# Veason-silverbullet/DIGAT

Measured on NVIDIA B200. Metric: impressions_scored_per_sec, higher is better.
Workload: dtype f32

## Files before the change

### digat_b200/csrc/gemm_tcgen05_persistent.cuh

```cuda
#pragma once
#include "gemm_tcgen05.cuh"
#include "gemm_tcgen05_pair.cuh"

namespace digat {

__device__ __forceinline__ void tma_load_2d_multicast(void* dst, const CUtensorMap* map, uint64_t* bar, int c0, int c1,
                                                      uint16_t cta_mask) {
    asm volatile(
        "cp.async.bulk.tensor.2d.shared::cluster.global.mbarrier::complete_tx::bytes.multicast::cluster [%0], [%1, {%3, %4}], [%2], %5;"
        :: "r"(smem_u32(dst)), "l"(reinterpret_cast<uint64_t>(map)), "r"(smem_u32(bar)), "r"(c0), "r"(c1), "h"(cta_mask) : "memory");
}
__device__ __forceinline__ void umma_commit_multicast(uint64_t* bar, uint16_t cta_mask) {
    asm volatile("tcgen05.commit.cta_group::1.mbarrier::arrive::one.shared::cluster.multicast::cluster.b64 [%0], %1;"
                 :: "r"(smem_u32(bar)), "h"(cta_mask) : "memory");
}

__device__ __forceinline__ void umma_bf16_2cta(uint32_t tmem_d, uint64_t da, uint64_t db, uint32_t idesc, uint32_t accumulate) {
    asm volatile(
        "{\n\t.reg .pred p;\n\t"
        "setp.ne.b32 p, %4, 0;\n\t"
        "tcgen05.mma.cta_group::2.kind::f16 [%0], %1, %2, %3, p;\n\t}"
        :: "r"(tmem_d), "l"(da), "l"(db), "r"(idesc), "r"(accumulate) : "memory");
}

constexpr int kTcEpiWarps = 8;
constexpr int kTcPersistThreads = (2 + 4 + kTcEpiWarps) * 32;

template <int BN, int kCl = 1>
struct TcPersistCfg {
    static constexpr int A_BYTES = 128 * kTcBK * 4;
    static constexpr int W_ROWS = kCl == 3 ? BN / 2 : BN;
    static constexpr int W_BYTES = W_ROWS * kTcBK * 4;
    static constexpr int STAGE_BYTES = 2 * A_BYTES + 2 * W_BYTES;
    static constexpr int MAX_N = 1280;
    static constexpr int GB_GROUPS = 16;
    static constexpr int EXTRA = 512  + MAX_N * 4 + kTcEpiWarps * 32 * 20 * 4  + GB_GROUPS * BN * 4;
    static constexpr int STAGES = (226 * 1024 - EXTRA) / STAGE_BYTES > 6 ? 6 : (226 * 1024 - EXTRA) / STAGE_BYTES;
    static constexpr int TMEM_COLS = 2 * BN <= 256 ? 256 : 512;
    static constexpr size_t SMEM = (size_t)STAGES * STAGE_BYTES + EXTRA;
    static_assert(STAGES >= 3, "not enough shared memory for the pipeline");
    static_assert(A_BYTES % 512 == 0 && W_BYTES % 512 == 0, "operand tiles must start on a swizzle-atom boundary");
};

template <int BN, bool kBf16, int kCl>
__global__ void __launch_bounds__(kTcPersistThreads, 1)
gemm_tf32x3_persistent_kernel(const __grid_constant__ CUtensorMap map_a, const __grid_constant__ CUtensorMap map_whi,
                              const __grid_constant__ CUtensorMap map_wlo, const __grid_constant__ CUtensorMap map_w3,
                              const float* __restrict__ bias,
                              float* __restrict__ C, int ldc, int M, int N, int K, GroupBias gb) {
    using Cfg = TcPersistCfg<BN, kCl>;
    extern __shared__ __align__(1024) uint8_t smem_raw[];
    uint8_t* smem = smem_raw;
    uint64_t* bars = reinterpret_cast<uint64_t*>(smem + (size_t)Cfg::STAGES * Cfg::STAGE_BYTES);
    uint64_t* full = bars;
    uint64_t* ready = bars + Cfg::STAGES;
    uint64_t* empty = bars + 2 * Cfg::STAGES;
    uint64_t* accum_full = bars + 3 * Cfg::STAGES;
    uint64_t* tmem_empty = accum_full + 1;
    uint64_t* peer_full = tmem_empty + 1;
    uint32_t* tmem_slot = reinterpret_cast<uint32_t*>(peer_full + Cfg::STAGES);
    float* bias_s = reinterpret_cast<float*>(smem + (size_t)Cfg::STAGES * Cfg::STAGE_BYTES + 512);
    float* stage_base = bias_s + Cfg::MAX_N;
    float* gb_s = stage_base + kTcEpiWarps * 32 * 20;

    const int warp = threadIdx.x >> 5, lane = threadIdx.x & 31;
    const int nkb_all = (K + kTcBK - 1) / kTcBK;
    const int nkb = (nkb_all + gb.kbatches - 1) / gb.kbatches;
    const int n_tiles_n = (N + BN - 1) / BN, n_tiles_m = (M + 127) / 128;
    const int cl_rank = kCl >= 2 ? (int)cluster_ctarank() : 0;
    const int worker = kCl >= 2 ? (int)(blockIdx.x >> 1) : (int)blockIdx.x;
    const int n_workers = kCl >= 2 ? (int)(gridDim.x >> 1) : (int)gridDim.x;
    const int n_units_m = kCl >= 2 ? (n_tiles_m + 1) / 2 : n_tiles_m;
    const int n_tiles_mn = n_tiles_n * n_units_m;
    const int n_tiles = n_tiles_mn * gb.kbatches;
    auto tile_mb = [&](int t_mn) { const int u = t_mn / n_tiles_n; return kCl >= 2 ? 2 * u + cl_rank : u; };
    auto tile_nb = [&](int t_mn) { return t_mn % n_tiles_n; };

    auto a_hi = [&](int s) { return smem + (size_t)s * Cfg::STAGE_BYTES; };
    auto a_lo = [&](int s) { return smem + (size_t)s * Cfg::STAGE_BYTES + Cfg::A_BYTES; };
    auto w_hi = [&](int s) { return smem + (size_t)s * Cfg::STAGE_BYTES + 2 * Cfg::A_BYTES; };
    auto w_lo = [&](int s) { return smem + (size_t)s * Cfg::STAGE_BYTES + 2 * Cfg::A_BYTES + Cfg::W_BYTES; };
    auto a_b2 = [&](int s) { return a_lo(s) + Cfg::A_BYTES / 2; };
    auto w_b3 = [&](int s) { return w_lo(s) + Cfg::W_BYTES / 2; };

    for (int i = threadIdx.x; i < N; i += kTcPersistThreads) bias_s[i] = bias != nullptr ? bias[i] : 0.f;
    if (warp == 0 && lane == 0) {
        asm volatile("prefetch.tensormap [%0];" :: "l"(reinterpret_cast<uint64_t>(&map_a)) : "memory");
        asm volatile("prefetch.tensormap [%0];" :: "l"(reinterpret_cast<uint64_t>(&map_whi)) : "memory");
        asm volatile("prefetch.tensormap [%0];" :: "l"(reinterpret_cast<uint64_t>(&map_wlo)) : "memory");
        for (int s = 0; s < Cfg::STAGES; ++s) {
            mbar_init(&full[s], 1);
            mbar_init(&ready[s], kTcTransformThreads / 32 + ((kCl == 3 && cl_rank == 0) ? 1 : 0));
            mbar_init(&empty[s], kCl == 2 ? 2 : 1);
            mbar_init(&peer_full[s], 1);
        }
        mbar_init(accum_full, 1);
        mbar_init(tmem_empty, kCl == 3 ? 2 * kTcEpiWarps : kTcEpiWarps);
        asm volatile("fence.mbarrier_init.release.cluster;" ::: "memory");
    }
    if (warp == 1) {
        if (kCl == 3) {
            asm volatile("tcgen05.alloc.cta_group::2.sync.aligned.shared::cta.b32 [%0], %1;"
                         :: "r"(smem_u32(tmem_slot)), "r"((uint32_t)Cfg::TMEM_COLS) : "memory");
            asm volatile("tcgen05.relinquish_alloc_permit.cta_group::2.sync.aligned;" ::: "memory");
        } else {
            asm volatile("tcgen05.alloc.cta_group::1.sync.aligned.shared::cta.b32 [%0], %1;"
                         :: "r"(smem_u32(tmem_slot)), "r"((uint32_t)Cfg::TMEM_COLS) : "memory");
            asm volatile("tcgen05.relinquish_alloc_permit.cta_group::1.sync.aligned;" ::: "memory");
        }
    }
    asm volatile("tcgen05.fence::before_thread_sync;" ::: "memory");
    if (kCl >= 2) cluster_sync_all();
    else __syncthreads();
    asm volatile("tcgen05.fence::after_thread_sync;" ::: "memory");
    const uint32_t tmem_base = *tmem_slot;

    if (warp == 0) {
        if (lane == 0) {
            int it = 0;
            for (int tile = worker; tile < n_tiles; tile += n_workers) {
                const int slice = tile / n_tiles_mn, t_mn = tile - slice * n_tiles_mn;
                const int mb = tile_mb(t_mn), m0 = mb * 128, n0 = tile_nb(t_mn) * BN;
                const int kb0 = slice * nkb;
                if (n0 == 0 && gb.kbatches == 1) {
                    const int ahead = mb + kTcPrefetchBlocks;
                    if (ahead < n_tiles_m)
                        for (int kb = 0; kb < nkb; ++kb)
                            asm volatile("cp.async.bulk.prefetch.tensor.2d.L2.global [%0, {%1, %2}];"
                                         :: "l"(reinterpret_cast<uint64_t>(&map_a)), "r"(kb * kTcBK), "r"(ahead * 128) : "memory");
                }
                for (int kb = 0; kb < nkb; ++kb, ++it) {
                    const int s = it % Cfg::STAGES;
                    if (kCl >= 2) mbar_wait_cluster(&empty[s], ((it / Cfg::STAGES) & 1) ^ 1);
                    else mbar_wait(&empty[s], ((it / Cfg::STAGES) & 1) ^ 1);
                    mbar_arrive_expect_tx(&full[s], Cfg::A_BYTES + 2 * Cfg::W_BYTES);
                    tma_load_2d(a_hi(s), &map_a, &full[s], (kb0 + kb) * kTcBK, m0);
                    if (kCl == 2) {
                        constexpr int HR = BN / 2;
                        const int nr = n0 + cl_rank * HR;
                        tma_load_2d_multicast(w_hi(s) + cl_rank * HR * kTcBK * 4, &map_whi, &full[s], (kb0 + kb) * kTcBK, nr, 3);
                        tma_load_2d_multicast(w_lo(s) + cl_rank * HR * kTcBK * (kBf16 ? 2 : 4), &map_wlo, &full[s], (kb0 + kb) * kTcBK, nr, 3);
                        if (kBf16) tma_load_2d_multicast(w_b3(s) + cl_rank * HR * kTcBK * 2, &map_w3, &full[s], (kb0 + kb) * kTcBK, nr, 3);
                    } else {
                        const int nr = kCl == 3 ? n0 + cl_rank * (BN / 2) : n0;
                        tma_load_2d(w_hi(s), &map_whi, &full[s], (kb0 + kb) * kTcBK, nr);
                        tma_load_2d(w_lo(s), &map_wlo, &full[s], (kb0 + kb) * kTcBK, nr);
                        if (kBf16) tma_load_2d(w_b3(s), &map_w3, &full[s], (kb0 + kb) * kTcBK, nr);
                    }
                }
            }
        }
    } else if (warp == 1) {
        if (kCl == 3) {
            if (lane == 0 && cl_rank == 0) {
                constexpr uint32_t idesc2 = umma_idesc_tf32(256, BN);
                constexpr uint32_t idesc2h = umma_idesc_bf16(256, BN);
                const uint32_t d_main = tmem_base, d_corr = tmem_base + (uint32_t)BN;
                int it = 0, j = 0;
                for (int tile = worker; tile < n_tiles; tile += n_workers, ++j) {
                    if (j > 0) {
                        mbar_wait_cluster(tmem_empty, (uint32_t)(j - 1) & 1u);
                        asm volatile("tcgen05.fence::after_thread_sync;" ::: "memory");
                    }
                    auto issue_raw = [&](int kb, int g) {
                        const int s = g % Cfg::STAGES;
                        mbar_wait(&full[s], (g / Cfg::STAGES) & 1);
                        mbar_wait_cluster(&peer_full[s], (g / Cfg::STAGES) & 1);
                        asm volatile("tcgen05.fence::after_thread_sync;" ::: "memory");
                        const uint64_t d_ahi = umma_desc_sw64(smem_u32(a_hi(s)));
                        const uint64_t d_whi = umma_desc_sw64(smem_u32(w_hi(s))), d_wlo = umma_desc_sw64(smem_u32(w_lo(s)));
#pragma unroll
                        for (int k = 0; k < kTcBK / 8; ++k) {
                            const uint64_t koff = (uint64_t)((k * 8 * 4) >> 4);
                            const uint32_t first = (kb > 0 || k > 0) ? 1u : 0u;
                            umma_tf32_2cta(d_main, d_ahi + koff, d_whi + koff, idesc2, first);
                            if (!kBf16) umma_tf32_2cta(d_corr, d_ahi + koff, d_wlo + koff, idesc2, first);
                        }
                    };
                    auto issue_lo = [&](int g) {
                        const int s = g % Cfg::STAGES;
                        mbar_wait_cluster(&ready[s], (g / Cfg::STAGES) & 1);
                        asm volatile("tcgen05.fence::after_thread_sync;" ::: "memory");
                        if (kBf16) {
                            const uint32_t first = (g - it) > 0 ? 1u : 0u;
                            umma_bf16_2cta(d_corr, umma_desc_sw32(smem_u32(a_lo(s))), umma_desc_sw32(smem_u32(w_b3(s))), idesc2h, first);
                            umma_bf16_2cta(d_corr, umma_desc_sw32(smem_u32(a_b2(s))), umma_desc_sw32(smem_u32(w_lo(s))), idesc2h, 1u);
                        } else {
                            const uint64_t d_alo = umma_desc_sw64(smem_u32(a_lo(s))), d_whi = umma_desc_sw64(smem_u32(w_hi(s)));
#pragma unroll
                            for (int k = 0; k < kTcBK / 8; ++k) {
                                const uint64_t koff = (uint64_t)((k * 8 * 4) >> 4);
                                umma_tf32_2cta(d_corr, d_alo + koff, d_whi + koff, idesc2, 1u);
                            }
                        }
                        umma_commit_2cta(&empty[s]);
                    };
                    issue_raw(0, it);
                    for (int kb = 0; kb < nkb; ++kb) {
                        if (kb + 1 < nkb) issue_raw(kb + 1, it + kb + 1);
                        issue_lo(it + kb);
                    }
                    it += nkb;
                    umma_commit_2cta(accum_full);
                }
            } else if (cl_rank == 1 && lane < 2) {
                int it = 0;
                for (int tile = worker; tile < n_tiles; tile += n_workers)
                    for (int kb = 0; kb < nkb; ++kb, ++it) {
                        const int s = it % Cfg::STAGES;
                        if (lane == 0) {
                            mbar_wait(&full[s], (it / Cfg::STAGES) & 1);
                            mbar_arrive_cluster(&peer_full[s], 0);
                        } else {
                            mbar_wait(&ready[s], (it / Cfg::STAGES) & 1);
                            mbar_arrive_cluster(&ready[s], 0);
                        }
                    }
            }
        } else if (lane == 0) {
            constexpr uint32_t idesc = umma_idesc_tf32(128, BN);
            const uint32_t d_main = tmem_base, d_corr = tmem_base + (uint32_t)BN;
            int it = 0, j = 0;
            for (int tile = worker; tile < n_tiles; tile += n_workers, ++j) {
#ifdef DIGAT_TC_TIMING
                const long long t0 = clock64();
#endif
                if (j > 0) {
                    mbar_wait(tmem_empty, (uint32_t)(j - 1) & 1u);
                    asm volatile("tcgen05.fence::after_thread_sync;" ::: "memory");
                }
#ifdef DIGAT_TC_TIMING
                const long long t1 = clock64();
#endif
                auto issue_raw = [&](int kb, int g) {
                    const int s = g % Cfg::STAGES;
                    mbar_wait(&full[s], (g / Cfg::STAGES) & 1);
                    asm volatile("tcgen05.fence::after_thread_sync;" ::: "memory");
                    const uint64_t d_ahi = umma_desc_sw64(smem_u32(a_hi(s)));
                    const uint64_t d_whi = umma_desc_sw64(smem_u32(w_hi(s))), d_wlo = umma_desc_sw64(smem_u32(w_lo(s)));
#pragma unroll
                    for (int k = 0; k < kTcBK / 8; ++k) {
                        const uint64_t koff = (uint64_t)((k * 8 * 4) >> 4);
                        const uint32_t first = (kb > 0 || k > 0) ? 1u : 0u;
                        umma_tf32(d_main, d_ahi + koff, d_whi + koff, idesc, first);
                        if (!kBf16) umma_tf32(d_corr, d_ahi + koff, d_wlo + koff, idesc, first);
                    }
                };
                auto issue_lo = [&](int g) {
                    const int s = g % Cfg::STAGES;
                    mbar_wait(&ready[s], (g / Cfg::STAGES) & 1);
                    asm volatile("tcgen05.fence::after_thread_sync;" ::: "memory");
                    if (kBf16) {
                        constexpr uint32_t idesc16 = umma_idesc_bf16(128, BN);
                        const uint32_t first = (g - it) > 0 ? 1u : 0u;
                        umma_bf16(d_corr, umma_desc_sw32(smem_u32(a_lo(s))), umma_desc_sw32(smem_u32(w_b3(s))), idesc16, first);
                        umma_bf16(d_corr, umma_desc_sw32(smem_u32(a_b2(s))), umma_desc_sw32(smem_u32(w_lo(s))), idesc16, 1u);
                    } else {
                        const uint64_t d_alo = umma_desc_sw64(smem_u32(a_lo(s))), d_whi = umma_desc_sw64(smem_u32(w_hi(s)));
#pragma unroll
                        for (int k = 0; k < kTcBK / 8; ++k) {
                            const uint64_t koff = (uint64_t)((k * 8 * 4) >> 4);
                            umma_tf32(d_corr, d_alo + koff, d_whi + koff, idesc, 1u);
                        }
                    }
                    if (kCl == 2) umma_commit_multicast(&empty[s], 3);
                    else umma_commit(&empty[s]);
                };
                issue_raw(0, it);
                for (int kb = 0; kb < nkb; ++kb) {
                    if (kb + 1 < nkb) issue_raw(kb + 1, it + kb + 1);
                    issue_lo(it + kb);
                }
                it += nkb;
                umma_commit(accum_full);
#ifdef DIGAT_TC_TIMING
                if (blockIdx.x == 7 && j >= 3 && j <= 5)
                    printf("mma  tile j=%d: waited tmem_empty %lld, issue loop %lld (abs %lld)\n", j, t1 - t0, clock64() - t1, t0);
#endif
            }
        }
    } else if (warp < 6) {
        const int t = threadIdx.x - 64;
        int it = 0;
        for (int tile = worker; tile < n_tiles; tile += n_workers) {
            for (int kb = 0; kb < nkb; ++kb, ++it) {
                const int s = it % Cfg::STAGES;
                mbar_wait(&full[s], (it / Cfg::STAGES) & 1);
                const float4* hi = reinterpret_cast<const float4*>(a_hi(s));
                float4* lo = reinterpret_cast<float4*>(a_lo(s));
#pragma unroll
                for (int i = 0; i < Cfg::A_BYTES / 16 / kTcTransformThreads; ++i) {
                    const int idx = t + i * kTcTransformThreads;
                    const float4 v = hi[idx];
                    if (kBf16) {
                        const int r = idx >> 2, c = (idx & 3) ^ ((r >> 1) & 3);
                        const uint32_t off = (uint32_t)(r * 32 + (((c >> 1) ^ ((r >> 2) & 1)) << 4) + ((c & 1) << 3));
                        __nv_bfloat162 p0 = __floats2bfloat162_rn(v.x, v.y), p1 = __floats2bfloat162_rn(v.z, v.w);
                        __nv_bfloat162 q0 = __floats2bfloat162_rn(v.x - tf32_trunc(v.x), v.y - tf32_trunc(v.y));
                        __nv_bfloat162 q1 = __floats2bfloat162_rn(v.z - tf32_trunc(v.z), v.w - tf32_trunc(v.w));
                        uint2 full_v, lo_v;
                        full_v.x = *reinterpret_cast<uint32_t*>(&p0); full_v.y = *reinterpret_cast<uint32_t*>(&p1);
                        lo_v.x = *reinterpret_cast<uint32_t*>(&q0); lo_v.y = *reinterpret_cast<uint32_t*>(&q1);
                        *reinterpret_cast<uint2*>(a_lo(s) + off) = full_v;
                        *reinterpret_cast<uint2*>(a_b2(s) + off) = lo_v;
                    } else {
                        float4 vl;
                        vl.x = to_tf32_rna(v.x - tf32_trunc(v.x)); vl.y = to_tf32_rna(v.y - tf32_trunc(v.y));
                        vl.z = to_tf32_rna(v.z - tf32_trunc(v.z)); vl.w = to_tf32_rna(v.w - tf32_trunc(v.w));
                        lo[idx] = vl;
                    }
                }
                asm volatile("fence.proxy.async.shared::cta;" ::: "memory");
                __syncwarp();
                if (lane == 0) mbar_arrive(&ready[s]);
            }
        }
    } else {
        const int q = warp & 3;
        const int ew = warp - 6;
        const int c_begin = (kTcEpiWarps == 8 && ew >= 4) ? (BN > 128 ? 128 : BN) : 0;
        const int c_end = (kTcEpiWarps == 8 && ew < 4) ? (BN > 128 ? 128 : BN) : BN;
        const bool has_gb = gb.ptr != nullptr;
        float* stage = stage_base + ew * (32 * 20);
        const uint32_t tbase = tmem_base + ((uint32_t)(q * 32) << 16);
        int j = 0;
        for (int tile = worker; tile < n_tiles; tile += n_workers, ++j) {
            const int slice = tile / n_tiles_mn, t_mn = tile - slice * n_tiles_mn;
            const int mb = tile_mb(t_mn), m0 = mb * 128, n0 = tile_nb(t_mn) * BN;
            float* __restrict__ Cs = C + (size_t)slice * (size_t)gb.c_batch_stride;
            const int m = m0 + q * 32 + lane;
            const int32_t* orow = gb.out_rows;
            const int mo = orow != nullptr ? orow[min(m, M - 1)] : m;
            const int g0 = has_gb ? (orow != nullptr ? orow[m0] : m0) / gb.rows : 0;
            const int g1 = has_gb ? (orow != nullptr ? orow[min(m0 + 127, M - 1)] : min(m0 + 127, M - 1)) / gb.rows : 0;
            const bool gb_tile = has_gb && n0 < gb.col0 + gb.cols && n0 + BN > gb.col0;
            const bool gb_smem = gb_tile && (g1 - g0 + 1) <= Cfg::GB_GROUPS;
            if (gb_smem) {
                asm volatile("bar.sync 1, %0;" :: "n"(kTcEpiWarps * 32) : "memory");
                const int te = threadIdx.x - 192;
                for (int idx = te; idx < (g1 - g0 + 1) * (BN / 4); idx += kTcEpiWarps * 32) {
                    const int gi = idx / (BN / 4), cq = idx - gi * (BN / 4);
                    const int col = n0 + cq * 4;
                    float4 v = make_float4(0.f, 0.f, 0.f, 0.f);
                    if (col >= gb.col0 && col < gb.col0 + gb.cols)
                        v = *reinterpret_cast<const float4*>(gb.ptr + (size_t)(g0 + gi) * gb.ld + (col - gb.col0));
                    *reinterpret_cast<float4*>(gb_s + gi * BN + cq * 4) = v;
                }
                asm volatile("bar.sync 1, %0;" :: "n"(kTcEpiWarps * 32) : "memory");
            }
            const float* grow = (gb_tile && !gb_smem && m < M) ? gb.ptr + (size_t)(mo / gb.rows) * gb.ld - gb.col0 + n0 : nullptr;
            const float* gsrow = gb_smem ? gb_s + ((orow != nullptr ? mo : min(m, M - 1)) / gb.rows - g0) * BN : nullptr;
#ifdef DIGAT_TC_TIMING
            const long long e0 = clock64();
#endif
            mbar_wait(accum_full, (uint32_t)j & 1u);
            asm volatile("tcgen05.fence::after_thread_sync;" ::: "memory");
#ifdef DIGAT_TC_TIMING
            const long long e1 = clock64();
#endif
            uint32_t rm[16], rc[16];
            float4 gq[4];
            auto issue_group = [&](int c) {
                asm volatile(
                    "tcgen05.ld.sync.aligned.32x32b.x16.b32 {%0,%1,%2,%3,%4,%5,%6,%7,%8,%9,%10,%11,%12,%13,%14,%15}, [%16];"
                    : "=r"(rm[0]), "=r"(rm[1]), "=r"(rm[2]), "=r"(rm[3]), "=r"(rm[4]), "=r"(rm[5]), "=r"(rm[6]), "=r"(rm[7]),
                      "=r"(rm[8]), "=r"(rm[9]), "=r"(rm[10]), "=r"(rm[11]), "=r"(rm[12]), "=r"(rm[13]), "=r"(rm[14]), "=r"(rm[15])
                    : "r"(tbase + (uint32_t)c));
                asm volatile(
                    "tcgen05.ld.sync.aligned.32x32b.x16.b32 {%0,%1,%2,%3,%4,%5,%6,%7,%8,%9,%10,%11,%12,%13,%14,%15}, [%16];"
                    : "=r"(rc[0]), "=r"(rc[1]), "=r"(rc[2]), "=r"(rc[3]), "=r"(rc[4]), "=r"(rc[5]), "=r"(rc[6]), "=r"(rc[7]),
                      "=r"(rc[8]), "=r"(rc[9]), "=r"(rc[10]), "=r"(rc[11]), "=r"(rc[12]), "=r"(rc[13]), "=r"(rc[14]), "=r"(rc[15])
                    : "r"(tbase + (uint32_t)(BN + c)));
#pragma unroll
                for (int v4 = 0; v4 < 4; ++v4) {
                    const int col = n0 + c + v4 * 4;
                    gq[v4] = (grow != nullptr && col >= gb.col0 && col < gb.col0 + gb.cols)
                                 ? *reinterpret_cast<const float4*>(grow + c + v4 * 4) : make_float4(0.f, 0.f, 0.f, 0.f);
                }
            };
            if (c_begin < c_end) {
                issue_group(c_begin);
            } else if (lane == 0) {
                if (kCl == 3 && cl_rank == 1) mbar_arrive_cluster(tmem_empty, 0);
                else mbar_arrive(tmem_empty);
            }
#pragma unroll 1
            for (int c = c_begin; c < c_end; c += 16) {
                asm volatile("tcgen05.wait::ld.sync.aligned;" ::: "memory");
                float o[16];
#pragma unroll
                for (int i = 0; i < 16; ++i)
                    o[i] = (__uint_as_float(rm[i]) + __uint_as_float(rc[i])) + ((n0 + c + i < N && slice == 0) ? bias_s[n0 + c + i] : 0.f);
#pragma unroll
                for (int v4 = 0; v4 < 4; ++v4) {
                    float4 gv = gq[v4];
                    if (gsrow != nullptr) gv = *reinterpret_cast<const float4*>(gsrow + c + v4 * 4);
                    o[v4 * 4 + 0] += gv.x; o[v4 * 4 + 1] += gv.y;
                    o[v4 * 4 + 2] += gv.z; o[v4 * 4 + 3] += gv.w;
                }
                if (c + 16 < c_end) {
                    issue_group(c + 16);
                } else {
                    asm volatile("tcgen05.fence::before_thread_sync;" ::: "memory");
                    __syncwarp();
                    if (lane == 0) {
                        if (kCl == 3 && cl_rank == 1) mbar_arrive_cluster(tmem_empty, 0);
                        else mbar_arrive(tmem_empty);
                    }
                }
                __syncwarp();
#pragma unroll
                for (int v4 = 0; v4 < 4; ++v4)
                    *reinterpret_cast<float4*>(stage + lane * 20 + v4 * 4) =
                        make_float4(o[v4 * 4 + 0], o[v4 * 4 + 1], o[v4 * 4 + 2], o[v4 * 4 + 3]);
                __syncwarp();
#pragma unroll
                for (int t4 = 0; t4 < 4; ++t4) {
                    const int f = t4 * 32 + lane, row = f >> 2, cq = f & 3;
                    const int mr = m0 + q * 32 + row;
                    const int mc = __shfl_sync(0xffffffffu, mo, row);
                    if (mr < M && n0 + c + cq * 4 < N)
                        *reinterpret_cast<float4*>(Cs + (size_t)mc * ldc + n0 + c + cq * 4) =
                            *reinterpret_cast<const float4*>(stage + row * 20 + cq * 4);
                }
            }
#ifdef DIGAT_TC_TIMING
            if (blockIdx.x == 7 && j >= 3 && j <= 5 && threadIdx.x == 192)
                printf("epi  tile j=%d: waited accum_full %lld, epilogue %lld (abs %lld)\n", j, e1 - e0, clock64() - e1, e0);
#endif
        }
    }
    asm volatile("tcgen05.fence::before_thread_sync;" ::: "memory");
    if (kCl >= 2) cluster_sync_all();
    else __syncthreads();
    if (warp == 1) {
        if (kCl == 3)
            asm volatile("tcgen05.dealloc.cta_group::2.sync.aligned.b32 %0, %1;"
                         :: "r"(tmem_base), "r"((uint32_t)Cfg::TMEM_COLS) : "memory");
        else
            asm volatile("tcgen05.dealloc.cta_group::1.sync.aligned.b32 %0, %1;"
                         :: "r"(tmem_base), "r"((uint32_t)Cfg::TMEM_COLS) : "memory");
    }
}

static int g_tc_cluster = 0;

template <int BN, bool kBf16, int kCl>
int launch_tf32x3_persistent_inst(const CUtensorMap& ma, const CUtensorMap& mh, const CUtensorMap& ml, const CUtensorMap& m3,
                                  const float* bias, float* C, int ldc, int M, int N, int K, GroupBias gb, int units, int sm_count,
                                  cudaStream_t st) {
    using Cfg = TcPersistCfg<BN, kCl>;
    auto kernel = gemm_tf32x3_persistent_kernel<BN, kBf16, kCl>;
    if (int rc_ = ensure_dynamic_smem(kernel, (size_t)Cfg::SMEM)) return rc_;
    if (kCl == 1) {
        const int grid = units < sm_count ? units : sm_count;
        kernel<<<grid, kTcPersistThreads, Cfg::SMEM, st>>>(ma, mh, ml, m3, bias, C, ldc, M, N, K, gb);
        return check_launch("digat_linear_tf32x3(persistent)");
    }
    cudaLaunchConfig_t cfg{};
    cfg.blockDim = dim3(kTcPersistThreads);
    cfg.dynamicSmemBytes = Cfg::SMEM;
    cfg.stream = st;
    cudaLaunchAttribute attr[1];
    attr[0].id = cudaLaunchAttributeClusterDimension;
    attr[0].val.clusterDim.x = 2;
    attr[0].val.clusterDim.y = 1;
    attr[0].val.clusterDim.z = 1;
    cfg.attrs = attr;
    cfg.numAttrs = 1;
    static int max_clusters[16] = {0};
    int dev = 0;
    DIGAT_CUDA(cudaGetDevice(&dev));
    if (dev >= 0 && dev < 16 && max_clusters[dev] == 0) {
        cfg.gridDim = dim3(2 * (sm_count / 2));
        int n = 0;
        DIGAT_CUDA(cudaOccupancyMaxActiveClusters(&n, kernel, &cfg));
        max_clusters[dev] = n > 0 ? n : -1;
    }
    int clusters = sm_count / 2;
    if (dev >= 0 && dev < 16 && max_clusters[dev] > 0 && max_clusters[dev] < clusters) clusters = max_clusters[dev];
    if (units < clusters) clusters = units;
    cfg.gridDim = dim3(2 * clusters);
    DIGAT_CUDA(cudaLaunchKernelEx(&cfg, kernel, ma, mh, ml, m3, bias, C, ldc, M, N, K, gb));
    return check_launch("digat_linear_tf32x3(persistent, W multicast)");
}

template <int BN>
int launch_tf32x3_persistent(const float* A, int lda, const float* W_hi, const float* W_lo, int ldw, const float* bias,
                             float* C, int ldc, int M, int N, int K, GroupBias gb, cudaStream_t st,
                             const void* W_hb, const void* W_lb) {
    using Cfg = TcPersistCfg<BN>;
    const DeviceInfo* di = device_info();
    if (!di) return fail(DIGAT_E_CUDA, "digat_linear_tf32x3: no CUDA device");
    DIGAT_REQUIRE(N <= Cfg::MAX_N, "digat_linear_tf32x3(persistent): N=%d exceeds %d", N, Cfg::MAX_N);
    const int tiles_n = (N + BN - 1) / BN, tiles_m = (M + 127) / 128;
    const bool cluster = g_tc_cluster != 0 && gb.kbatches == 1 && tiles_m >= 2 && (BN / 2) % 8 == 0 &&
                         (long)tiles_n * tiles_m >= 4L * di->sm_count;
    const int wbox = cluster ? BN / 2 : BN;
    CUtensorMap ma, mh, ml;
    int rc;
    if ((rc = make_tensor_map_2d(&ma, A, M, K, lda, 128, kTcBK, CU_TENSOR_MAP_SWIZZLE_64B)) != DIGAT_OK) return rc;
    if ((rc = make_tensor_map_2d(&mh, W_hi, N, K, ldw, wbox, kTcBK, CU_TENSOR_MAP_SWIZZLE_64B)) != DIGAT_OK) return rc;
    const bool bf16c = W_hb != nullptr && W_lb != nullptr;
    CUtensorMap m3 = mh;
    if (bf16c) {
        if ((rc = make_tensor_map_2d_bf16(&ml, W_hb, N, K, ldw, wbox, kTcBK, CU_TENSOR_MAP_SWIZZLE_32B)) != DIGAT_OK) return rc;
        if ((rc = make_tensor_map_2d_bf16(&m3, W_lb, N, K, ldw, wbox, kTcBK, CU_TENSOR_MAP_SWIZZLE_32B)) != DIGAT_OK) return rc;
    } else {
        if ((rc = make_tensor_map_2d(&ml, W_lo, N, K, ldw, wbox, kTcBK, CU_TENSOR_MAP_SWIZZLE_64B)) != DIGAT_OK) return rc;
    }
    const int units = tiles_n * (cluster ? (tiles_m + 1) / 2 : tiles_m) * gb.kbatches;
    if (cluster && g_tc_cluster == 2) {
        if (bf16c) return launch_tf32x3_persistent_inst<BN, true, 3>(ma, mh, ml, m3, bias, C, ldc, M, N, K, gb, units, di->sm_count, st);
        return launch_tf32x3_persistent_inst<BN, false, 3>(ma, mh, ml, m3, bias, C, ldc, M, N, K, gb, units, di->sm_count, st);
    }
    if (cluster) {
        if (bf16c) return launch_tf32x3_persistent_inst<BN, true, 2>(ma, mh, ml, m3, bias, C, ldc, M, N, K, gb, units, di->sm_count, st);
        return launch_tf32x3_persistent_inst<BN, false, 2>(ma, mh, ml, m3, bias, C, ldc, M, N, K, gb, units, di->sm_count, st);
    }
    if (bf16c) return launch_tf32x3_persistent_inst<BN, true, 1>(ma, mh, ml, m3, bias, C, ldc, M, N, K, gb, units, di->sm_count, st);
    return launch_tf32x3_persistent_inst<BN, false, 1>(ma, mh, ml, m3, bias, C, ldc, M, N, K, gb, units, di->sm_count, st);
}

}
```

Baseline: 753,000.

## Drain whole TMEM accumulator into registers early and rebalance warp registers

The warp layout becomes 16 warps split into a producer/MMA warpgroup, a transform warpgroup and 8 epilogue warps. setmaxnreg moves registers from the first two groups to the epilogue group. Each epilogue warp now loads its full half of the main and correction accumulators from TMEM into registers, sums them, and releases tmem_empty before doing bias, residual and stores. This lets the MMA warp start the next tile sooner, at the cost of high register pressure in the epilogue and possible spills. Timing instrumentation is also extended.

```diff
diff --git a/digat_b200/csrc/gemm_tcgen05_persistent.cuh b/digat_b200/csrc/gemm_tcgen05_persistent.cuh
--- a/digat_b200/csrc/gemm_tcgen05_persistent.cuh
+++ b/digat_b200/csrc/gemm_tcgen05_persistent.cuh
@@ -23,8 +23,43 @@
         :: "r"(tmem_d), "l"(da), "l"(db), "r"(idesc), "r"(accumulate) : "memory");
 }
 
+__device__ __forceinline__ void tmem_ld16(uint32_t taddr, uint32_t* r) {
+    asm volatile(
+        "tcgen05.ld.sync.aligned.32x32b.x16.b32 {%0,%1,%2,%3,%4,%5,%6,%7,%8,%9,%10,%11,%12,%13,%14,%15}, [%16];"
+        : "=r"(r[0]), "=r"(r[1]), "=r"(r[2]), "=r"(r[3]), "=r"(r[4]), "=r"(r[5]), "=r"(r[6]), "=r"(r[7]),
+          "=r"(r[8]), "=r"(r[9]), "=r"(r[10]), "=r"(r[11]), "=r"(r[12]), "=r"(r[13]), "=r"(r[14]), "=r"(r[15])
+        : "r"(taddr));
+}
+__device__ __forceinline__ void tmem_ld8(uint32_t taddr, uint32_t* r) {
+    asm volatile("tcgen05.ld.sync.aligned.32x32b.x8.b32 {%0,%1,%2,%3,%4,%5,%6,%7}, [%8];"
+                 : "=r"(r[0]), "=r"(r[1]), "=r"(r[2]), "=r"(r[3]), "=r"(r[4]), "=r"(r[5]), "=r"(r[6]), "=r"(r[7])
+                 : "r"(taddr));
+}
+__device__ __forceinline__ void tmem_tie(uint32_t* r, int n) {
+#pragma unroll
+    for (int i = 0; i < n; ++i) asm volatile("" : "+r"(r[i]));
+}
+template <int NC, int C0>
+__device__ __forceinline__ void tmem_add_corr(uint32_t tcorr, uint32_t* s) {
+    constexpr int n = NC - C0 < 32 ? NC - C0 : 32;
+    uint32_t t[32];
+#pragma unroll
+    for (int c = 0; c < n; c += 16) {
+        if (n - c >= 16) tmem_ld16(tcorr + (uint32_t)(C0 + c), t + c);
+        else tmem_ld8(tcorr + (uint32_t)(C0 + c), t + c);
+    }
+    asm volatile("tcgen05.wait::ld.sync.aligned;" ::: "memory");
+    tmem_tie(t, n);
+    if (C0 == 0) tmem_tie(s, NC);
+#pragma unroll
+    for (int i = 0; i < n; ++i) s[C0 + i] = __float_as_uint(__uint_as_float(s[C0 + i]) + __uint_as_float(t[i]));
+    if constexpr (C0 + 32 < NC) tmem_add_corr<NC, C0 + 32>(tcorr, s);
+}
+
 constexpr int kTcEpiWarps = 8;
-constexpr int kTcPersistThreads = (2 + 4 + kTcEpiWarps) * 32;
+constexpr int kTcPersistThreads = 16 * 32;
+constexpr int kTcRegsWg0 = 56, kTcRegsTransform = 56, kTcRegsEpi = 200;
+static_assert(128 * kTcRegsWg0 + 128 * kTcRegsTransform + 256 * kTcRegsEpi == 65536, "register budgets must fill the SM");
 
 template <int BN, int kCl = 1>
 struct TcPersistCfg {
@@ -115,57 +150,138 @@
     asm volatile("tcgen05.fence::after_thread_sync;" ::: "memory");
     const uint32_t tmem_base = *tmem_slot;
 
-    if (warp == 0) {
-        if (lane == 0) {
-            int it = 0;
-            for (int tile = worker; tile < n_tiles; tile += n_workers) {
-                const int slice = tile / n_tiles_mn, t_mn = tile - slice * n_tiles_mn;
-                const int mb = tile_mb(t_mn), m0 = mb * 128, n0 = tile_nb(t_mn) * BN;
-                const int kb0 = slice * nkb;
-                if (n0 == 0 && gb.kbatches == 1) {
-                    const int ahead = mb + kTcPrefetchBlocks;
-                    if (ahead < n_tiles_m)
-                        for (int kb = 0; kb < nkb; ++kb)
-                            asm volatile("cp.async.bulk.prefetch.tensor.2d.L2.global [%0, {%1, %2}];"
-                                         :: "l"(reinterpret_cast<uint64_t>(&map_a)), "r"(kb * kTcBK), "r"(ahead * 128) : "memory");
-                }
-                for (int kb = 0; kb < nkb; ++kb, ++it) {
-                    const int s = it % Cfg::STAGES;
-                    if (kCl >= 2) mbar_wait_cluster(&empty[s], ((it / Cfg::STAGES) & 1) ^ 1);
-                    else mbar_wait(&empty[s], ((it / Cfg::STAGES) & 1) ^ 1);
-                    mbar_arrive_expect_tx(&full[s], Cfg::A_BYTES + 2 * Cfg::W_BYTES);
-                    tma_load_2d(a_hi(s), &map_a, &full[s], (kb0 + kb) * kTcBK, m0);
-                    if (kCl == 2) {
-                        constexpr int HR = BN / 2;
-                        const int nr = n0 + cl_rank * HR;
-                        tma_load_2d_multicast(w_hi(s) + cl_rank * HR * kTcBK * 4, &map_whi, &full[s], (kb0 + kb) * kTcBK, nr, 3);
-                        tma_load_2d_multicast(w_lo(s) + cl_rank * HR * kTcBK * (kBf16 ? 2 : 4), &map_wlo, &full[s], (kb0 + kb) * kTcBK, nr, 3);
-                        if (kBf16) tma_load_2d_multicast(w_b3(s) + cl_rank * HR * kTcBK * 2, &map_w3, &full[s], (kb0 + kb) * kTcBK, nr, 3);
-                    } else {
-                        const int nr = kCl == 3 ? n0 + cl_rank * (BN / 2) : n0;
-                        tma_load_2d(w_hi(s), &map_whi, &full[s], (kb0 + kb) * kTcBK, nr);
-                        tma_load_2d(w_lo(s), &map_wlo, &full[s], (kb0 + kb) * kTcBK, nr);
-                        if (kBf16) tma_load_2d(w_b3(s), &map_w3, &full[s], (kb0 + kb) * kTcBK, nr);
+    if (warp < 4) {
+        asm volatile("setmaxnreg.dec.sync.aligned.u32 %0;" :: "n"(kTcRegsWg0));
+        if (warp == 0) {
+            if (lane == 0) {
+                int it = 0;
+                for (int tile = worker; tile < n_tiles; tile += n_workers) {
+                    const int slice = tile / n_tiles_mn, t_mn = tile - slice * n_tiles_mn;
+                    const int mb = tile_mb(t_mn), m0 = mb * 128, n0 = tile_nb(t_mn) * BN;
+                    const int kb0 = slice * nkb;
+                    if (n0 == 0 && gb.kbatches == 1) {
+                        const int ahead = mb + kTcPrefetchBlocks;
+                        if (ahead < n_tiles_m)
+                            for (int kb = 0; kb < nkb; ++kb)
+                                asm volatile("cp.async.bulk.prefetch.tensor.2d.L2.global [%0, {%1, %2}];"
+                                             :: "l"(reinterpret_cast<uint64_t>(&map_a)), "r"(kb * kTcBK), "r"(ahead * 128) : "memory");
                     }
-                }
-            }
-        }
-    } else if (warp == 1) {
-        if (kCl == 3) {
-            if (lane == 0 && cl_rank == 0) {
-                constexpr uint32_t idesc2 = umma_idesc_tf32(256, BN);
-                constexpr uint32_t idesc2h = umma_idesc_bf16(256, BN);
+                    for (int kb = 0; kb < nkb; ++kb, ++it) {
+                        const int s = it % Cfg::STAGES;
+                        if (kCl >= 2) mbar_wait_cluster(&empty[s], ((it / Cfg::STAGES) & 1) ^ 1);
+                        else mbar_wait(&empty[s], ((it / Cfg::STAGES) & 1) ^ 1);
+                        mbar_arrive_expect_tx(&full[s], Cfg::A_BYTES + 2 * Cfg::W_BYTES);
+                        tma_load_2d(a_hi(s), &map_a, &full[s], (kb0 + kb) * kTcBK, m0);
+                        if (kCl == 2) {
+                            constexpr int HR = BN / 2;
+                            const int nr = n0 + cl_rank * HR;
+                            tma_load_2d_multicast(w_hi(s) + cl_rank * HR * kTcBK * 4, &map_whi, &full[s], (kb0 + kb) * kTcBK, nr, 3);
+                            tma_load_2d_multicast(w_lo(s) + cl_rank * HR * kTcBK * (kBf16 ? 2 : 4), &map_wlo, &full[s], (kb0 + kb) * kTcBK, nr, 3);
+                            if (kBf16) tma_load_2d_multicast(w_b3(s) + cl_rank * HR * kTcBK * 2, &map_w3, &full[s], (kb0 + kb) * kTcBK, nr, 3);
+                        } else {
+                            const int nr = kCl == 3 ? n0 + cl_rank * (BN / 2) : n0;
+                            tma_load_2d(w_hi(s), &map_whi, &full[s], (kb0 + kb) * kTcBK, nr);
+                            tma_load_2d(w_lo(s), &map_wlo, &full[s], (kb0 + kb) * kTcBK, nr);
+                            if (kBf16) tma_load_2d(w_b3(s), &map_w3, &full[s], (kb0 + kb) * kTcBK, nr);
+                        }
+                    }
+                }
+            }
+        } else if (warp == 1) {
+            if (kCl == 3) {
+                if (lane == 0 && cl_rank == 0) {
+                    constexpr uint32_t idesc2 = umma_idesc_tf32(256, BN);
+                    constexpr uint32_t idesc2h = umma_idesc_bf16(256, BN);
+                    const uint32_t d_main = tmem_base, d_corr = tmem_base + (uint32_t)BN;
+                    int it = 0, j = 0;
+                    for (int tile = worker; tile < n_tiles; tile += n_workers, ++j) {
+                        if (j > 0) {
+                            mbar_wait_cluster(tmem_empty, (uint32_t)(j - 1) & 1u);
+                            asm volatile("tcgen05.fence::after_thread_sync;" ::: "memory");
+                        }
+                        auto issue_raw = [&](int kb, int g) {
+                            const int s = g % Cfg::STAGES;
+                            mbar_wait(&full[s], (g / Cfg::STAGES) & 1);
+                            mbar_wait_cluster(&peer_full[s], (g / Cfg::STAGES) & 1);
+                            asm volatile("tcgen05.fence::after_thread_sync;" ::: "memory");
+                            const uint64_t d_ahi = umma_desc_sw64(smem_u32(a_hi(s)));
+                            const uint64_t d_whi = umma_desc_sw64(smem_u32(w_hi(s))), d_wlo = umma_desc_sw64(smem_u32(w_lo(s)));
+#pragma unroll
+                            for (int k = 0; k < kTcBK / 8; ++k) {
+                                const uint64_t koff = (uint64_t)((k * 8 * 4) >> 4);
+                                const uint32_t first = (kb > 0 || k > 0) ? 1u : 0u;
+                                umma_tf32_2cta(d_main, d_ahi + koff, d_whi + koff, idesc2, first);
+                                if (!kBf16) umma_tf32_2cta(d_corr, d_ahi + koff, d_wlo + koff, idesc2, first);
+                            }
+                        };
+                        auto issue_lo = [&](int g) {
+                            const int s = g % Cfg::STAGES;
+                            mbar_wait_cluster(&ready[s], (g / Cfg::STAGES) & 1);
+                            asm volatile("tcgen05.fence::after_thread_sync;" ::: "memory");
+                            if (kBf16) {
+                                const uint32_t first = (g - it) > 0 ? 1u : 0u;
+                                umma_bf16_2cta(d_corr, umma_desc_sw32(smem_u32(a_lo(s))), umma_desc_sw32(smem_u32(w_b3(s))), idesc2h, first);
+                                umma_bf16_2cta(d_corr, umma_desc_sw32(smem_u32(a_b2(s))), umma_desc_sw32(smem_u32(w_lo(s))), idesc2h, 1u);
+                            } else {
+                                const uint64_t d_alo = umma_desc_sw64(smem_u32(a_lo(s))), d_whi = umma_desc_sw64(smem_u32(w_hi(s)));
+#pragma unroll
+                                for (int k = 0; k < kTcBK / 8; ++k) {
+                                    const uint64_t koff = (uint64_t)((k * 8 * 4) >> 4);
+                                    umma_tf32_2cta(d_corr, d_alo + koff, d_whi + koff, idesc2, 1u);
+                                }
+                            }
+                            umma_commit_2cta(&empty[s]);
+                        };
+                        issue_raw(0, it);
+                        for (int kb = 0; kb < nkb; ++kb) {
+                            if (kb + 1 < nkb) issue_raw(kb + 1, it + kb + 1);
+                            issue_lo(it + kb);
+                        }
+                        it += nkb;
+                        umma_commit_2cta(accum_full);
+                    }
+                } else if (cl_rank == 1 && lane < 2) {
+                    int it = 0;
+                    for (int tile = worker; tile < n_tiles; tile += n_workers)
+                        for (int kb = 0; kb < nkb; ++kb, ++it) {
+                            const int s = it % Cfg::STAGES;
+                            if (lane == 0) {
+                                mbar_wait(&full[s], (it / Cfg::STAGES) & 1);
+                                mbar_arrive_cluster(&peer_full[s], 0);
+                            } else {
+                                mbar_wait(&ready[s], (it / Cfg::STAGES) & 1);
+                                mbar_arrive_cluster(&ready[s], 0);
+                            }
+                        }
+                }
+            } else if (lane == 0) {
+                constexpr uint32_t idesc = umma_idesc_tf32(128, BN);
                 const uint32_t d_main = tmem_base, d_corr = tmem_base + (uint32_t)BN;
                 int it = 0, j = 0;
+#ifdef DIGAT_TC_TIMING
+                long long s_tmem = 0, s_full = 0, s_ready = 0, s_loop = 0, k_start = clock64();
+                unsigned long long g_start; asm volatile("mov.u64 %0, %%globaltimer;" : "=l"(g_start));
+#endif
                 for (int tile = worker; tile < n_tiles; tile += n_workers, ++j) {
+#ifdef DIGAT_TC_TIMING
+                    const long long t0 = clock64();
+#endif
                     if (j > 0) {
-                        mbar_wait_cluster(tmem_empty, (uint32_t)(j - 1) & 1u);
+                        mbar_wait(tmem_empty, (uint32_t)(j - 1) & 1u);
                         asm volatile("tcgen05.fence::after_thread_sync;" ::: "memory");
                     }
+#ifdef DIGAT_TC_TIMING
+                    const long long t1 = clock64();
+#endif
                     auto issue_raw = [&](int kb, int g) {
                         const int s = g % Cfg::STAGES;
+#ifdef DIGAT_TC_TIMING
+                        const long long w0 = clock64();
+#endif
                         mbar_wait(&full[s], (g / Cfg::STAGES) & 1);
-                        mbar_wait_cluster(&peer_full[s], (g / Cfg::STAGES) & 1);
+#ifdef DIGAT_TC_TIMING
+                        s_full += clock64() - w0;
+#endif
                         asm volatile("tcgen05.fence::after_thread_sync;" ::: "memory");
                         const uint64_t d_ahi = umma_desc_sw64(smem_u32(a_hi(s)));
                         const uint64_t d_whi = umma_desc_sw64(smem_u32(w_hi(s))), d_wlo = umma_desc_sw64(smem_u32(w_lo(s)));
@@ -173,27 +289,35 @@
                         for (int k = 0; k < kTcBK / 8; ++k) {
                             const uint64_t koff = (uint64_t)((k * 8 * 4) >> 4);
                             const uint32_t first = (kb > 0 || k > 0) ? 1u : 0u;
-                            umma_tf32_2cta(d_main, d_ahi + koff, d_whi + koff, idesc2, first);
-                            if (!kBf16) umma_tf32_2cta(d_corr, d_ahi + koff, d_wlo + koff, idesc2, first);
+                            umma_tf32(d_main, d_ahi + koff, d_whi + koff, idesc, first);
+                            if (!kBf16) umma_tf32(d_corr, d_ahi + koff, d_wlo + koff, idesc, first);
                         }
                     };
                     auto issue_lo = [&](int g) {
                         const int s = g % Cfg::STAGES;
-                        mbar_wait_cluster(&ready[s], (g / Cfg::STAGES) & 1);
+#ifdef DIGAT_TC_TIMING
+                        const long long w0 = clock64();
+#endif
+                        mbar_wait(&ready[s], (g / Cfg::STAGES) & 1);
+#ifdef DIGAT_TC_TIMING
+                        s_ready += clock64() - w0;
+#endif
                         asm volatile("tcgen05.fence::after_thread_sync;" ::: "memory");
                         if (kBf16) {
+                            constexpr uint32_t idesc16 = umma_idesc_bf16(128, BN);
                             const uint32_t first = (g - it) > 0 ? 1u : 0u;
-                            umma_bf16_2cta(d_corr, umma_desc_sw32(smem_u32(a_lo(s))), umma_desc_sw32(smem_u32(w_b3(s))), idesc2h, first);
-                            umma_bf16_2cta(d_corr, umma_desc_sw32(smem_u32(a_b2(s))), umma_desc_sw32(smem_u32(w_lo(s))), idesc2h, 1u);
+                            umma_bf16(d_corr, umma_desc_sw32(smem_u32(a_lo(s))), umma_desc_sw32(smem_u32(w_b3(s))), idesc16, first);
+                            umma_bf16(d_corr, umma_desc_sw32(smem_u32(a_b2(s))), umma_desc_sw32(smem_u32(w_lo(s))), idesc16, 1u);
                         } else {
                             const uint64_t d_alo = umma_desc_sw64(smem_u32(a_lo(s))), d_whi = umma_desc_sw64(smem_u32(w_hi(s)));
 #pragma unroll
                             for (int k = 0; k < kTcBK / 8; ++k) {
                                 const uint64_t koff = (uint64_t)((k * 8 * 4) >> 4);
-                                umma_tf32_2cta(d_corr, d_alo + koff, d_whi + koff, idesc2, 1u);
+                                umma_tf32(d_corr, d_alo + koff, d_whi + koff, idesc, 1u);
                             }
                         }
-                        umma_commit_2cta(&empty[s]);
+                        if (kCl == 2) umma_commit_multicast(&empty[s], 3);
+                        else umma_commit(&empty[s]);
                     };
                     issue_raw(0, it);
                     for (int kb = 0; kb < nkb; ++kb) {
@@ -201,86 +325,23 @@
                         issue_lo(it + kb);
                     }
                     it += nkb;
-                    umma_commit_2cta(accum_full);
-                }
-            } else if (cl_rank == 1 && lane < 2) {
-                int it = 0;
-                for (int tile = worker; tile < n_tiles; tile += n_workers)
-                    for (int kb = 0; kb < nkb; ++kb, ++it) {
-                        const int s = it % Cfg::STAGES;
-                        if (lane == 0) {
-                            mbar_wait(&full[s], (it / Cfg::STAGES) & 1);
-                            mbar_arrive_cluster(&peer_full[s], 0);
-                        } else {
-                            mbar_wait(&ready[s], (it / Cfg::STAGES) & 1);
-                            mbar_arrive_cluster(&ready[s], 0);
-                        }
-                    }
-            }
-        } else if (lane == 0) {
-            constexpr uint32_t idesc = umma_idesc_tf32(128, BN);
-            const uint32_t d_main = tmem_base, d_corr = tmem_base + (uint32_t)BN;
-            int it = 0, j = 0;
-            for (int tile = worker; tile < n_tiles; tile += n_workers, ++j) {
-#ifdef DIGAT_TC_TIMING
-                const long long t0 = clock64();
-#endif
-                if (j > 0) {
-                    mbar_wait(tmem_empty, (uint32_t)(j - 1) & 1u);
-                    asm volatile("tcgen05.fence::after_thread_sync;" ::: "memory");
-                }
-#ifdef DIGAT_TC_TIMING
-                const long long t1 = clock64();
-#endif
-                auto issue_raw = [&](int kb, int g) {
-                    const int s = g % Cfg::STAGES;
-                    mbar_wait(&full[s], (g / Cfg::STAGES) & 1);
-                    asm volatile("tcgen05.fence::after_thread_sync;" ::: "memory");
-                    const uint64_t d_ahi = umma_desc_sw64(smem_u32(a_hi(s)));
-                    const uint64_t d_whi = umma_desc_sw64(smem_u32(w_hi(s))), d_wlo = umma_desc_sw64(smem_u32(w_lo(s)));
-#pragma unroll
-                    for (int k = 0; k < kTcBK / 8; ++k) {
-                        const uint64_t koff = (uint64_t)((k * 8 * 4) >> 4);
-                        const uint32_t first = (kb > 0 || k > 0) ? 1u : 0u;
-                        umma_tf32(d_main, d_ahi + koff, d_whi + koff, idesc, first);
-                        if (!kBf16) umma_tf32(d_corr, d_ahi + koff, d_wlo + koff, idesc, first);
-                    }
-                };
-                auto issue_lo = [&](int g) {
-                    const int s = g % Cfg::STAGES;
-                    mbar_wait(&ready[s], (g / Cfg::STAGES) & 1);
-                    asm volatile("tcgen05.fence::after_thread_sync;" ::: "memory");
-                    if (kBf16) {
-                        constexpr uint32_t idesc16 = umma_idesc_bf16(128, BN);
-                        const uint32_t first = (g - it) > 0 ? 1u : 0u;
-                        umma_bf16(d_corr, umma_desc_sw32(smem_u32(a_lo(s))), umma_desc_sw32(smem_u32(w_b3(s))), idesc16, first);
-                        umma_bf16(d_corr, umma_desc_sw32(smem_u32(a_b2(s))), umma_desc_sw32(smem_u32(w_lo(s))), idesc16, 1u);
-                    } else {
-                        const uint64_t d_alo = umma_desc_sw64(smem_u32(a_lo(s))), d_whi = umma_desc_sw64(smem_u32(w_hi(s)));
-#pragma unroll
-                        for (int k = 0; k < kTcBK / 8; ++k) {
-                            const uint64_t koff = (uint64_t)((k * 8 * 4) >> 4);
-                            umma_tf32(d_corr, d_alo + koff, d_whi + koff, idesc, 1u);
-                        }
-                    }
-                    if (kCl == 2) umma_commit_multicast(&empty[s], 3);
-                    else umma_commit(&empty[s]);
-                };
-                issue_raw(0, it);
-                for (int kb = 0; kb < nkb; ++kb) {
-                    if (kb + 1 < nkb) issue_raw(kb + 1, it + kb + 1);
-                    issue_lo(it + kb);
-                }
-                it += nkb;
-                umma_commit(accum_full);
-#ifdef DIGAT_TC_TIMING
-                if (blockIdx.x == 7 && j >= 3 && j <= 5)
-                    printf("mma  tile j=%d: waited tmem_empty %lld, issue loop %lld (abs %lld)\n", j, t1 - t0, clock64() - t1, t0);
+                    umma_commit(accum_full);
+#ifdef DIGAT_TC_TIMING
+                    s_tmem += t1 - t0; s_loop += clock64() - t1;
+#endif
+                }
+#ifdef DIGAT_TC_TIMING
+                unsigned long long g_end; asm volatile("mov.u64 %0, %%globaltimer;" : "=l"(g_end));
+                if (blockIdx.x % 37 == 7)
+                    printf("mma cta %d, %d tiles: %lld cycles (%llu ns -> %.0f MHz), waited tmem_empty %lld, issue loop %lld (waited full %lld, ready %lld)\n",
+                           blockIdx.x, j, clock64() - k_start, g_end - g_start, (clock64() - k_start) * 1e3 / (double)(g_end - g_start),
+                           s_tmem, s_loop, s_full, s_ready);
 #endif
             }
         }
-    } else if (warp < 6) {
-        const int t = threadIdx.x - 64;
+    } else if (warp < 8) {
+        asm volatile("setmaxnreg.dec.sync.aligned.u32 %0;" :: "n"(kTcRegsTransform));
+        const int t = threadIdx.x - 128;
         int it = 0;
         for (int tile = worker; tile < n_tiles; tile += n_workers) {
             for (int kb = 0; kb < nkb; ++kb, ++it) {
@@ -316,14 +377,19 @@
             }
         }
     } else {
+        asm volatile("setmaxnreg.inc.sync.aligned.u32 %0;" :: "n"(kTcRegsEpi));
+        constexpr int CW = BN / 2;
+        static_assert(CW % 8 == 0, "an epilogue warp's columns are drained and stored 8 at a time");
         const int q = warp & 3;
-        const int ew = warp - 6;
-        const int c_begin = (kTcEpiWarps == 8 && ew >= 4) ? (BN > 128 ? 128 : BN) : 0;
-        const int c_end = (kTcEpiWarps == 8 && ew < 4) ? (BN > 128 ? 128 : BN) : BN;
+        const int ew = warp - 8;
+        const int c0 = ew < 4 ? 0 : CW;
         const bool has_gb = gb.ptr != nullptr;
         float* stage = stage_base + ew * (32 * 20);
-        const uint32_t tbase = tmem_base + ((uint32_t)(q * 32) << 16);
+        const uint32_t tbase = tmem_base + ((uint32_t)(q * 32) << 16) + (uint32_t)c0;
         int j = 0;
+#ifdef DIGAT_TC_TIMING
+        long long s_accum = 0, s_drain = 0, s_epi = 0;
+#endif
         for (int tile = worker; tile < n_tiles; tile += n_workers, ++j) {
             const int slice = tile / n_tiles_mn, t_mn = tile - slice * n_tiles_mn;
             const int mb = tile_mb(t_mn), m0 = mb * 128, n0 = tile_nb(t_mn) * BN;
@@ -337,7 +403,7 @@
             const bool gb_smem = gb_tile && (g1 - g0 + 1) <= Cfg::GB_GROUPS;
             if (gb_smem) {
                 asm volatile("bar.sync 1, %0;" :: "n"(kTcEpiWarps * 32) : "memory");
-                const int te = threadIdx.x - 192;
+                const int te = threadIdx.x - 256;
                 for (int idx = te; idx < (g1 - g0 + 1) * (BN / 4); idx += kTcEpiWarps * 32) {
                     const int gi = idx / (BN / 4), cq = idx - gi * (BN / 4);
                     const int col = n0 + cq * 4;
@@ -358,65 +424,47 @@
 #ifdef DIGAT_TC_TIMING
             const long long e1 = clock64();
 #endif
-            uint32_t rm[16], rc[16];
-            float4 gq[4];
-            auto issue_group = [&](int c) {
-                asm volatile(
-                    "tcgen05.ld.sync.aligned.32x32b.x16.b32 {%0,%1,%2,%3,%4,%5,%6,%7,%8,%9,%10,%11,%12,%13,%14,%15}, [%16];"
-                    : "=r"(rm[0]), "=r"(rm[1]), "=r"(rm[2]), "=r"(rm[3]), "=r"(rm[4]), "=r"(rm[5]), "=r"(rm[6]), "=r"(rm[7]),
-                      "=r"(rm[8]), "=r"(rm[9]), "=r"(rm[10]), "=r"(rm[11]), "=r"(rm[12]), "=r"(rm[13]), "=r"(rm[14]), "=r"(rm[15])
-                    : "r"(tbase + (uint32_t)c));
-                asm volatile(
-                    "tcgen05.ld.sync.aligned.32x32b.x16.b32 {%0,%1,%2,%3,%4,%5,%6,%7,%8,%9,%10,%11,%12,%13,%14,%15}, [%16];"
-                    : "=r"(rc[0]), "=r"(rc[1]), "=r"(rc[2]), "=r"(rc[3]), "=r"(rc[4]), "=r"(rc[5]), "=r"(rc[6]), "=r"(rc[7]),
-                      "=r"(rc[8]), "=r"(rc[9]), "=r"(rc[10]), "=r"(rc[11]), "=r"(rc[12]), "=r"(rc[13]), "=r"(rc[14]), "=r"(rc[15])
-                    : "r"(tbase + (uint32_t)(BN + c)));
-#pragma unroll
-                for (int v4 = 0; v4 < 4; ++v4) {
-                    const int col = n0 + c + v4 * 4;
-                    gq[v4] = (grow != nullptr && col >= gb.col0 && col < gb.col0 + gb.cols)
-                                 ? *reinterpret_cast<const float4*>(grow + c + v4 * 4) : make_float4(0.f, 0.f, 0.f, 0.f);
-                }
-            };
-            if (c_begin < c_end) {
-                issue_group(c_begin);
-            } else if (lane == 0) {
+            uint32_t s[CW];
+#pragma unroll
+            for (int c = 0; c < CW; c += 16) {
+                if (CW - c >= 16) tmem_ld16(tbase + (uint32_t)c, s + c);
+                else tmem_ld8(tbase + (uint32_t)c, s + c);
+            }
+            tmem_add_corr<CW, 0>(tbase + (uint32_t)BN, s);
+            asm volatile("tcgen05.fence::before_thread_sync;" ::: "memory");
+            __syncwarp();
+            if (lane == 0) {
                 if (kCl == 3 && cl_rank == 1) mbar_arrive_cluster(tmem_empty, 0);
                 else mbar_arrive(tmem_empty);
             }
-#pragma unroll 1
-            for (int c = c_begin; c < c_end; c += 16) {
-                asm volatile("tcgen05.wait::ld.sync.aligned;" ::: "memory");
-                float o[16];
-#pragma unroll
-                for (int i = 0; i < 16; ++i)
-                    o[i] = (__uint_as_float(rm[i]) + __uint_as_float(rc[i])) + ((n0 + c + i < N && slice == 0) ? bias_s[n0 + c + i] : 0.f);
-#pragma unroll
-                for (int v4 = 0; v4 < 4; ++v4) {
-                    float4 gv = gq[v4];
+#ifdef DIGAT_TC_TIMING
+            const long long e2 = clock64();
+#endif
+#pragma unroll
+            for (int cl = 0; cl < CW; cl += 8) {
+                const int c = c0 + cl;
+                float o[8];
+#pragma unroll
+                for (int i = 0; i < 8; ++i)
+                    o[i] = __uint_as_float(s[cl + i]) + ((n0 + c + i < N && slice == 0) ? bias_s[n0 + c + i] : 0.f);
+#pragma unroll
+                for (int v4 = 0; v4 < 2; ++v4) {
+                    const int col = n0 + c + v4 * 4;
+                    float4 gv = (grow != nullptr && col >= gb.col0 && col < gb.col0 + gb.cols)
+                                    ? *reinterpret_cast<const float4*>(grow + c + v4 * 4) : make_float4(0.f, 0.f, 0.f, 0.f);
                     if (gsrow != nullptr) gv = *reinterpret_cast<const float4*>(gsrow + c + v4 * 4);
                     o[v4 * 4 + 0] += gv.x; o[v4 * 4 + 1] += gv.y;
                     o[v4 * 4 + 2] += gv.z; o[v4 * 4 + 3] += gv.w;
                 }
-                if (c + 16 < c_end) {
-                    issue_group(c + 16);
-                } else {
-                    asm volatile("tcgen05.fence::before_thread_sync;" ::: "memory");
-                    __syncwarp();
-                    if (lane == 0) {
-                        if (kCl == 3 && cl_rank == 1) mbar_arrive_cluster(tmem_empty, 0);
-                        else mbar_arrive(tmem_empty);
-                    }
-                }
                 __syncwarp();
 #pragma unroll
-                for (int v4 = 0; v4 < 4; ++v4)
+                for (int v4 = 0; v4 < 2; ++v4)
                     *reinterpret_cast<float4*>(stage + lane * 20 + v4 * 4) =
                         make_float4(o[v4 * 4 + 0], o[v4 * 4 + 1], o[v4 * 4 + 2], o[v4 * 4 + 3]);
                 __syncwarp();
 #pragma unroll
-                for (int t4 = 0; t4 < 4; ++t4) {
-                    const int f = t4 * 32 + lane, row = f >> 2, cq = f & 3;
+                for (int t4 = 0; t4 < 2; ++t4) {
+                    const int f = t4 * 32 + lane, row = f >> 1, cq = f & 1;
                     const int mr = m0 + q * 32 + row;
                     const int mc = __shfl_sync(0xffffffffu, mo, row);
                     if (mr < M && n0 + c + cq * 4 < N)
@@ -425,10 +473,14 @@
                 }
             }
 #ifdef DIGAT_TC_TIMING
-            if (blockIdx.x == 7 && j >= 3 && j <= 5 && threadIdx.x == 192)
-                printf("epi  tile j=%d: waited accum_full %lld, epilogue %lld (abs %lld)\n", j, e1 - e0, clock64() - e1, e0);
+            s_accum += e1 - e0; s_drain += e2 - e1; s_epi += clock64() - e1;
 #endif
         }
+#ifdef DIGAT_TC_TIMING
+        if (blockIdx.x % 37 == 7 && threadIdx.x == 256)
+            printf("epi cta %d, %d tiles: waited accum_full %lld, drain to tmem_empty %lld, epilogue %lld\n",
+                   blockIdx.x, j, s_accum, s_drain, s_epi);
+#endif
     }
     asm volatile("tcgen05.fence::before_thread_sync;" ::: "memory");
     if (kCl >= 2) cluster_sync_all();
```

After: 763,800, median of 6. No clear change (+1.4%).
